# tonyzyl/ladcast

Hardware: AMD Instinct MI355X
Metric: ensemble-member-steps/sec (higher is better)
Workload: dtype f32

## Files before the change

### ladcast_amd/csrc/gemm_bf16x3_v3.hip

```cpp
#include <math.h>
#include <stdio.h>
#include <stdlib.h>

#include "common.h"

namespace {

#include "gemm_v3_common.inc"
#include "gemm_v3_kstep_f32.inc"

struct SKArgs {
  DevProblem pr[MAXP];
  int np;
  int G;
  long long U;
  long long tiles;
  float* ws;
  unsigned* counters;
  unsigned upg, urem;
};

__device__ __forceinline__ long long range_start(long long g, const SKArgs& a) {
  const unsigned gu = static_cast<unsigned>(g);
  return static_cast<long long>(gu * a.upg + (gu < a.urem ? gu : a.urem));
}

__device__ __forceinline__ int find_problem_by_unit(const SKArgs& a, long long u) {
  int pi = 0;
#pragma unroll
  for (int k = 1; k < MAXP; ++k)
    if (k < a.np && u >= a.pr[k].unit0) pi = k;
  return pi;
}

#ifdef LDC_GEMM_STAMPS
#define LDC_STAMP(i)                                                                                        \
  if (threadIdx.x == 0)                                                                                     \
    reinterpret_cast<unsigned long long*>(a.counters)[65536 + blockIdx.x * 16 + (i)] = __builtin_amdgcn_s_memrealtime();
#define LDC_STAMP_CLK(i)                                                                                    \
  if (threadIdx.x == 0)                                                                                     \
    reinterpret_cast<unsigned long long*>(a.counters)[65536 + blockIdx.x * 16 + (i)] = __builtin_amdgcn_s_memtime();
#else
#define LDC_STAMP(i)
#define LDC_STAMP_CLK(i)
#endif

template <int BM, int TERMS, bool CONV = false>
__global__ __launch_bounds__(512) void gemm_bf16x3_v3_kernel(SKArgs a) {
  constexpr int CPK = TERMS == 1 ? 2 * BK : BK;
  constexpr int RT = BM / 128;
  constexpr int NACC = RT * 8;
  constexpr int STAGE_B = (BM + BN) * ROW_B;
  constexpr int SLOT_FLOATS = BM * BN;
  constexpr int NAI = BM / 64;
  constexpr int ND = NAI + 2;
  constexpr int NDH = ND / 2;
  extern __shared__ __attribute__((aligned(16))) unsigned char smem[];
  const int wave = __builtin_amdgcn_readfirstlane(static_cast<int>(threadIdx.x) >> 6);
  LDC_STAMP(0)
  int seg_ = 0;
  (void)seg_;
  int g;
  {
    const int bid = blockIdx.x, G = a.G;
    const int q = G >> 3, r = G & 7, xcd = bid & 7;
    g = (xcd < r ? xcd * (q + 1) : r * (q + 1) + (xcd - r) * q) + (bid >> 3);
  }
  auto uniform64 = [](long long v) {
    const unsigned lo = __builtin_amdgcn_readfirstlane(static_cast<unsigned>(v));
    const unsigned hi = __builtin_amdgcn_readfirstlane(static_cast<unsigned>(static_cast<unsigned long long>(v) >> 32));
    return static_cast<long long>((static_cast<unsigned long long>(hi) << 32) | lo);
  };
  const long long u_begin = uniform64(range_start(g, a));
  const long long u_end = uniform64(range_start(g + 1, a));
  const unsigned smem_lds = lds_addr(smem);

  struct Seg {
    int pi, tile, k0, k1, b, bm, bn;
  };
  auto decode = [&](long long u_) {
    Seg sg;
    sg.pi = find_problem_by_unit(a, u_);
    const DevProblem& Q = a.pr[sg.pi];
    const unsigned local = static_cast<unsigned>(u_ - Q.unit0), kt_u = static_cast<unsigned>(Q.kt);
    sg.tile = __builtin_amdgcn_readfirstlane(static_cast<int>(local / kt_u));
    sg.k0 = static_cast<int>(local - static_cast<unsigned>(sg.tile) * kt_u);
    const long long left = u_end - u_;
    sg.k1 = (Q.kt - sg.k0 <= left) ? Q.kt : sg.k0 + static_cast<int>(left);
    const unsigned per_b = static_cast<unsigned>(Q.tm * Q.tn), tile_u = static_cast<unsigned>(sg.tile);
    const unsigned b_ = tile_u / per_b;
    const unsigned t_in = tile_u - b_ * per_b;
    const unsigned strip = static_cast<unsigned>(Q.rm * Q.tn);
    const unsigned sr = t_in / strip;
    const unsigned r_in = t_in - sr * strip;
    const int rest = Q.tm - static_cast<int>(sr) * Q.rm;
    const unsigned h_sr = static_cast<unsigned>(rest < Q.rm ? rest : Q.rm);
    const unsigned bn_ = r_in / h_sr;
    sg.b = __builtin_amdgcn_readfirstlane(static_cast<int>(b_));
    sg.bn = __builtin_amdgcn_readfirstlane(static_cast<int>(bn_));
    sg.bm = __builtin_amdgcn_readfirstlane(static_cast<int>(sr) * Q.rm + static_cast<int>(r_in - bn_ * h_sr));
    return sg;
  };
  auto prefetch_next = [&](const Seg& sg) __attribute__((always_inline)) {
    const DevProblem& Q = a.pr[sg.pi];
    const int ln = fresh_lane();
    const int lr_ = ln >> 3, lp_ = ln & 7;
    const float* __restrict__ An = Q.A + static_cast<long long>(sg.b) * Q.d.a_bs;
    const long long wrb = static_cast<long long>(Q.d.K) * (TERMS == 1 ? 2 : 4);
    unsigned char* dump = smem + NSTAGE * STAGE_B + wave * 1024;
#pragma unroll
    for (int j = 0; j < 2; ++j) {
      const bool live = sg.k0 + j < sg.k1;
      const long long koff = static_cast<long long>(live ? sg.k0 + j : sg.k1 - 1) * (BK * 4);
      unsigned char* sA = smem + j * STAGE_B;
      unsigned char* sW = sA + BM * ROW_B;
#pragma unroll
      for (int i = 0; i < NAI; ++i) {
        const int r = 8 * (wave + 8 * i) + lr_;
        int gm = sg.bm * BM + r;
        gm = gm < Q.d.M ? gm : Q.d.M - 1;
        dma16(reinterpret_cast<const unsigned char*>(An + static_cast<long long>(gm) * Q.d.lda) + ((lp_ ^ swz(r)) << 4) + koff,
              live ? sA + (wave + 8 * i) * 1024 : dump);
      }
#pragma unroll
      for (int i = 0; i < 2; ++i) {
        const int r = 8 * (wave + 8 * i) + lr_;
        int gn = sg.bn * BN + r;
        gn = gn < Q.d.N ? gn : Q.d.N - 1;
        dma16(Q.W + static_cast<long long>(gn) * wrb + ((lp_ ^ swz(r)) << 4) + koff, live ? sW + (wave + 8 * (i)) * 1024 : dump);
      }
    }
  };
  long long u = u_begin;
  Seg cur{};
  if (u < u_end) cur = decode(u);
  bool prefetched = false;
  while (u < u_end) {
    const int pi = cur.pi;
    const DevProblem& P = a.pr[pi];
    const int tile = cur.tile, k0 = cur.k0, k1 = cur.k1, b = cur.b, bm = cur.bm, bn = cur.bn;
    const int lane = fresh_lane();
    const int fr = lane & 15;
    const int kg = lane >> 4;
    const int lr = lane >> 3, lp = lane & 7;
    const unsigned f_r = swz(fr);
    const unsigned off_hi = fr * ROW_B + (((2 * kg) ^ f_r) << 4);
    const unsigned off_lo = fr * ROW_B + (((2 * kg + 1) ^ f_r) << 4);
    const unsigned a_hi = smem_lds + (16 * RT * wave) * ROW_B + off_hi;
    const unsigned a_lo = smem_lds + (16 * RT * wave) * ROW_B + off_lo;
    const unsigned w_hi = smem_lds + BM * ROW_B + off_hi;
    const unsigned w_lo = smem_lds + BM * ROW_B + off_lo;
    const int M = P.d.M, N = P.d.N, K = P.d.K;
    const bool wave_rows = bm * BM + 16 * RT * wave < M;
    const float* __restrict__ A = P.A + static_cast<long long>(b) * P.d.a_bs;
    const int lda = P.d.lda;
    const long long w_row_bytes = static_cast<long long>(K) * (TERMS == 1 ? 2 : 4);

#ifdef LDC_GEMM_STAMPS_PROLOGUE
    if (seg_ == 0) { LDC_STAMP(9) }
#endif
    const unsigned char* a_src[NAI];
    const unsigned char* w_src[2];
    int pix_b[NAI], pix_hw[NAI];
    const int cslot = lp ^ swz(8 * (wave & 1) + lr);
    auto conv_tap_base = [&](int i, int tap) {
      const int ky = tap / P.ks, kx = tap - ky * P.ks;
      const int src = pix_b[i] + ldc_sphere_src_pixel(pix_hw[i] >> 16, pix_hw[i] & 0xffff, ky, kx, P.cH, P.cW, P.ks);
      return reinterpret_cast<const unsigned char*>(A + static_cast<long long>(src) * lda) + (cslot << 4);
    };
#pragma unroll
    for (int i = 0; i < NAI; ++i) {
      const int r = 8 * (wave + 8 * i) + lr;
      int gm = bm * BM + r;
      gm = gm < M ? gm : M - 1;
      if constexpr (CONV) {
        const int hw = P.cH * P.cW;
        const int bimg = gm / hw;
        const int rem = gm - bimg * hw;
        const int h = rem / P.cW;
        pix_b[i] = bimg * hw;
        pix_hw[i] = (h << 16) | (rem - h * P.cW);
        a_src[i] = conv_tap_base(i, k0 >> P.kshift);
      } else {
        a_src[i] = reinterpret_cast<const unsigned char*>(A + static_cast<long long>(gm) * lda) + ((lp ^ swz(r)) << 4);
      }
    }
#pragma unroll
    for (int i = 0; i < 2; ++i) {
      const int r = 8 * (wave + 8 * i) + lr;
      int gn = bn * BN + r;
      gn = gn < N ? gn : N - 1;
      w_src[i] = P.W + static_cast<long long>(gn) * w_row_bytes + ((lp ^ swz(r)) << 4);
    }
    auto issue_one = [&](int kt_, int stage, int i) {
      const bool live = kt_ < k1;
      unsigned char* sA = smem + stage * STAGE_B;
      unsigned char* sW = sA + BM * ROW_B;
      unsigned char* dump = smem + NSTAGE * STAGE_B + wave * 1024;
      const int kt = live ? kt_ : k1 - 1;
      const long long koff = static_cast<long long>(kt) * (BK * 4);
#ifdef LDC_GEMM_DIAG_NODMA
      if (kt >= 0) return;
#endif
      if (i < NAI) {
        if constexpr (CONV) {
          const int chunk = kt & ((1 << P.kshift) - 1);
          if (chunk == 0) a_src[i] = conv_tap_base(i, kt >> P.kshift);
          const unsigned char* src = a_src[i] + chunk * (BK * 4);
          if (chunk * CPK + CPK > P.cin) {
            if (chunk * CPK + (TERMS == 0 ? 4 * cslot : 8 * (TERMS == 3 ? (cslot >> 1) : cslot)) >= P.cin) src = P.zero16;
          }
          dma16(src, live ? sA + (wave + 8 * i) * 1024 : dump);
        } else {
          dma16(a_src[i] + koff, live ? sA + (wave + 8 * i) * 1024 : dump);
        }
      } else {
        dma16(w_src[i - NAI] + koff, live ? sW + (wave + 8 * (i - NAI)) * 1024 : dump);
      }
    };

    f32x4 acc[NACC];
#pragma unroll
    for (int i = 0; i < NACC; ++i) acc[i] = f32x4{0.f, 0.f, 0.f, 0.f};

    i32x4v wh0, wl0, wh1, wl1, wh2, wl2, wh3, wl3;
    i32x4v ah0[RT], al0[RT], ah1[RT], al1[RT];

#define LDC_SB __builtin_amdgcn_sched_barrier(0)
#define LDC_RD_W(WH, WL, SBH, SBL, CT)                                           \
  {                                                                              \
    LDC_DS_READ(WH, SBH, (CT) * (16 * ROW_B));                                   \
    LDC_DS_READ(WL, SBL, (CT) * (16 * ROW_B));                                   \
  }
#define LDC_RD_A(AH, AL, SBH, SBL)                                               \
  {                                                                              \
    LDC_DS_READ(AH[0], SBH, 0);                                                  \
    LDC_DS_READ(AL[0], SBL, 0);                                                  \
    if constexpr (RT == 2) {                                                     \
      LDC_DS_READ(AH[RT - 1], SBH, 16 * ROW_B);                                  \
      LDC_DS_READ(AL[RT - 1], SBL, 16 * ROW_B);                                  \
    }                                                                            \
  }
#define LDC_MM(ACC, WF, AF)                                                                                  \
  ACC = __builtin_amdgcn_mfma_f32_16x16x32_bf16(__builtin_bit_cast(bf16x8, WF), __builtin_bit_cast(bf16x8, AF), ACC, 0, 0, 0); \
  LDC_SB;
#define LDC_MMF(ACC, WF, AF, J)                                                                               \
  ACC = __builtin_amdgcn_mfma_f32_16x16x4f32(__int_as_float(WF[J]), __int_as_float(AF[J]), ACC, 0, 0, 0);     \
  LDC_SB;
#define LDC_CT(CT, WH, WL, AH, AL)                                               \
  if (wave_rows) {                                                               \
    if constexpr (TERMS == 0) {                                                  \
      _Pragma("unroll") for (int j_ = 0; j_ < 4; ++j_) {                         \
        LDC_MMF(acc[(CT)], WH, AH[0], j_)                                        \
        if constexpr (RT == 2) {                                                 \
          LDC_MMF(acc[8 + (CT)], WH, AH[RT - 1], j_)                             \
        }                                                                        \
      }                                                                          \
      _Pragma("unroll") for (int j_ = 0; j_ < 4; ++j_) {                         \
        LDC_MMF(acc[(CT)], WL, AL[0], j_)                                        \
        if constexpr (RT == 2) {                                                 \
          LDC_MMF(acc[8 + (CT)], WL, AL[RT - 1], j_)                             \
        }                                                                        \
      }                                                                          \
    } else if constexpr (TERMS == 1) {                                           \
      LDC_MM(acc[(CT)], WH, AH[0])                                               \
      if constexpr (RT == 2) {                                                   \
        LDC_MM(acc[8 + (CT)], WH, AH[RT - 1])                                    \
      }                                                                          \
      LDC_MM(acc[(CT)], WL, AL[0])                                               \
      if constexpr (RT == 2) {                                                   \
        LDC_MM(acc[8 + (CT)], WL, AL[RT - 1])                                    \
      }                                                                          \
    } else if constexpr (RT == 2) {                                              \
      LDC_MM(acc[(CT)], WH, AL[0])                                               \
      LDC_MM(acc[8 + (CT)], WH, AL[RT - 1])                                      \
      LDC_MM(acc[(CT)], WL, AH[0])                                               \
      LDC_MM(acc[8 + (CT)], WL, AH[RT - 1])                                      \
      LDC_MM(acc[(CT)], WH, AH[0])                                               \
      LDC_MM(acc[8 + (CT)], WH, AH[RT - 1])                                      \
    } else {                                                                     \
      LDC_MM(acc[(CT)], WH, AL[0])                                               \
      LDC_MM(acc[(CT)], WL, AH[0])                                               \
      LDC_MM(acc[(CT)], WH, AH[0])                                               \
    }                                                                            \
  }
#ifdef LDC_GEMM_DIAG_NOBARRIER
#define LDC_KSTEP_BARRIER
#else
#define LDC_KSTEP_BARRIER __builtin_amdgcn_s_barrier();
#endif
#define LDC_WAIT(N, X, Y)                                                        \
  asm volatile("s_waitcnt lgkmcnt(6)" : "+v"(X), "+v"(Y));                       \
  LDC_SB;
#define LDC_KSTEP(AH, AL, AHN, ALN)                                                                          \
  {                                                                                                          \
    const int st1 = st == NSTAGE - 1 ? 0 : st + 1;                                                           \
    const int st2 = st1 == NSTAGE - 1 ? 0 : st1 + 1;                                                         \
    const unsigned sb1 = st1 * STAGE_B;                                                                      \
    const unsigned wch = w_hi + sb, wcl = w_lo + sb, wnh = w_hi + sb1, wnl = w_lo + sb1;                     \
    const unsigned anh = a_hi + sb1, anl = a_lo + sb1;                                                       \
    constexpr bool dma2 = true;              \
    constexpr bool dma3 = true;  \
        \
    if constexpr (RT == 2) {                                                                                 \
      asm volatile("s_waitcnt lgkmcnt(6)" : "+v"(AH[0]), "+v"(AL[0]), "+v"(AH[1]), "+v"(AL[1]), "+v"(wh0), "+v"(wl0)); \
    } else {                                                                                                 \
      asm volatile("s_waitcnt lgkmcnt(6)" : "+v"(AH[0]), "+v"(AL[0]), "+v"(wh0), "+v"(wl0));                 \
    }                                                                                                        \
    LDC_SB;                                                                                                  \
    LDC_CT(0, wh0, wl0, AH, AL)                                                                              \
    LDC_RD_W(wh0, wl0, wch, wcl, 4)                                                                                \
    if (dma2) issue_one(kt + 2, st2, NDH + 0);                                                               \
    LDC_WAIT(6, wh1, wl1)                                                                                    \
    LDC_CT(1, wh1, wl1, AH, AL)                                                                              \
    LDC_RD_W(wh1, wl1, wch, wcl, 5)                                                                                \
    if (dma2) issue_one(kt + 2, st2, NDH + 1);                                                               \
    LDC_WAIT(6, wh2, wl2)                                                                                    \
    LDC_CT(2, wh2, wl2, AH, AL)                                                                              \
    LDC_RD_W(wh2, wl2, wch, wcl, 6)                                                                                \
    if constexpr (NDH == 3) {                                                                                \
      if (dma2) issue_one(kt + 2, st2, NDH + 2);                                                             \
    }                                                                                                        \
    LDC_WAIT(6, wh3, wl3)                                                                                    \
    LDC_CT(3, wh3, wl3, AH, AL)                                                                              \
    LDC_RD_W(wh3, wl3, wch, wcl, 7)                                                                          \
    LDC_WAIT(6, wh0, wl0)                                                                                    \
    LDC_CT(4, wh0, wl0, AH, AL)                                                                              \
                                                                         \
    asm volatile("s_waitcnt lgkmcnt(0)" : "+v"(wh1), "+v"(wl1), "+v"(wh2), "+v"(wl2), "+v"(wh3), "+v"(wl3)); \
    if constexpr (ND == 6) {                                                                                 \
      asm volatile("s_waitcnt vmcnt(6)" ::: "memory");                                                       \
    } else {                                                                                                 \
      asm volatile("s_waitcnt vmcnt(4)" ::: "memory");                                                       \
    }                                                                                                        \
    LDC_KSTEP_BARRIER                                                                                        \
    LDC_SB;                                                                                                  \
                          \
    LDC_RD_A(AHN, ALN, anh, anl)                                                                             \
    LDC_RD_W(wh0, wl0, wnh, wnl, 0)                                                                          \
    if (dma3) issue_one(kt + 3, st, 0);                                                                      \
    LDC_SB;                                                                                                  \
    LDC_CT(5, wh1, wl1, AH, AL)                                                                              \
    LDC_RD_W(wh1, wl1, wnh, wnl, 1)                                                                               \
    if (dma3) issue_one(kt + 3, st, 1);                                                                      \
    LDC_SB;                                                                                                  \
    LDC_CT(6, wh2, wl2, AH, AL)                                                                              \
    LDC_RD_W(wh2, wl2, wnh, wnl, 2)                                                                               \
    if constexpr (NDH == 3) {                                                                                \
      if (dma3) issue_one(kt + 3, st, 2);                                                                    \
    }                                                                                                        \
    LDC_SB;                                                                                                  \
    LDC_CT(7, wh3, wl3, AH, AL)                                                                              \
    LDC_RD_W(wh3, wl3, wnh, wnl, 3)                                                                               \
    LDC_SB;                                                                                                  \
    st = st1;                                                                                                \
    sb = sb1;                                                                                                \
  }

#define LDC_MM_ON(ACC, WF, AF, J) LDC_MMF(ACC, WF, AF, J)
#define LDC_MM_OFF(ACC, WF, AF, J)
#if defined(LDC_AB_BUILD) && defined(LDC_GEMM_F32_NO_PAIRS)
  constexpr bool PAIRED = false;
#else
  constexpr bool PAIRED = TERMS == 0 && RT == 1;
#endif

#ifdef LDC_GEMM_STAMPS_PROLOGUE
    if (seg_ == 0) { LDC_STAMP(10) }
#endif
    if (!prefetched) {
#pragma unroll
      for (int i = 0; i < ND; ++i) issue_one(k0, 0, i);
#pragma unroll
      for (int i = 0; i < ND; ++i) issue_one(k0 + 1, 1, i);
    }
#ifdef LDC_GEMM_STAMPS_PROLOGUE
    if (seg_ == 0) { LDC_STAMP(11) }
#endif
    const long long u_next = u + (k1 - k0);
    Seg nxt = cur;
    if (u_next < u_end) nxt = decode(u_next);
    if constexpr (ND == 6) {
      asm volatile("s_waitcnt vmcnt(6)" ::: "memory");
    } else {
      asm volatile("s_waitcnt vmcnt(4)" ::: "memory");
    }
    __builtin_amdgcn_s_barrier();
    LDC_STAMP(1 + 4 * seg_)
    if (seg_ == 0) { LDC_STAMP_CLK(13) }
    if constexpr (PAIRED) {
      LDC_KSTEP_Q_PROLOGUE(ah0, al0)
    } else {
      LDC_RD_A(ah0, al0, a_hi, a_lo)
      LDC_RD_W(wh0, wl0, w_hi, w_lo, 0)
      LDC_RD_W(wh1, wl1, w_hi, w_lo, 1)
      LDC_RD_W(wh2, wl2, w_hi, w_lo, 2)
      LDC_RD_W(wh3, wl3, w_hi, w_lo, 3)
    }
#pragma unroll
    for (int i = 0; i < NDH; ++i) issue_one(k0 + 2, 2, i);
    LDC_SB;

    unsigned sb = 0;
    int st = 0;
    if constexpr (PAIRED) {
      static_assert(!PAIRED || ND == 4, "the interleaved k-step is written for the 128-row tile's 4 DMA pieces");
      if (wave_rows) {
        for (int kt = k0; kt < k1; ++kt) {
          LDC_KSTEP_Q(ah0, al0, ah1, al1, LDC_MM_ON)
          ++kt;
          if (kt >= k1) break;
          LDC_KSTEP_Q(ah1, al1, ah0, al0, LDC_MM_ON)
        }
      } else {
        for (int kt = k0; kt < k1; ++kt) {
          LDC_KSTEP_Q(ah0, al0, ah1, al1, LDC_MM_OFF)
          ++kt;
          if (kt >= k1) break;
          LDC_KSTEP_Q(ah1, al1, ah0, al0, LDC_MM_OFF)
        }
      }
    } else {
      for (int kt = k0; kt < k1; ++kt) {
        LDC_KSTEP(ah0, al0, ah1, al1)
        ++kt;
        if (kt >= k1) break;
        LDC_KSTEP(ah1, al1, ah0, al0)
      }
    }
    asm volatile("s_waitcnt lgkmcnt(0)" : "+v"(wh0), "+v"(wl0), "+v"(wh1), "+v"(wl1), "+v"(wh2), "+v"(wl2), "+v"(wh3), "+v"(wl3));
#pragma unroll
    for (int rt = 0; rt < RT; ++rt) asm volatile("" : "+v"(ah0[rt]), "+v"(al0[rt]), "+v"(ah1[rt]), "+v"(al1[rt]));
#undef LDC_KSTEP
#undef LDC_MM_ON
#undef LDC_MM_OFF
#undef LDC_WAIT
#undef LDC_CT
#undef LDC_MMF
#undef LDC_MM
#undef LDC_RD_A
#undef LDC_RD_W
#undef LDC_SB
    __builtin_amdgcn_s_barrier();
    prefetched = false;
    if constexpr (!CONV && TERMS == 0) {
#if !defined(LDC_GEMM_DIAG_NODMA) && !defined(LDC_GEMM_NO_PREFETCH)
      if (u_next < u_end) {
        prefetch_next(nxt);
        prefetched = true;
      }
#endif
    }
    if (seg_ == 0) { LDC_STAMP_CLK(14) }
    LDC_STAMP(2 + 4 * seg_)

    if (k0 == 0 && k1 == P.kt) {
      tile_epilogue<BM, !CONV, LinearRows<BM>, true, TERMS == 0>(P, b, bm, bn, acc, wave, lane);
    } else {
      const int lane_h = fresh_lane();
      float* slot = a.ws + (static_cast<long long>(2 * g) + (k0 > 0 ? 0 : 1)) * SLOT_FLOATS + lane_h;
#pragma unroll
      for (int i = 0; i < NACC; ++i)
#pragma unroll
        for (int r = 0; r < 4; ++r)
          __hip_atomic_store(slot + ((wave * NACC + i) * 4 + r) * 64, acc[i][r], __ATOMIC_RELAXED, __HIP_MEMORY_SCOPE_AGENT);
      asm volatile("s_waitcnt vmcnt(0)" ::: "memory");
      __builtin_amdgcn_s_barrier();
      const long long f = P.unit0 + static_cast<long long>(tile) * P.kt;
      const long long l = f + P.kt;
      long long g_first = g;
      while (g_first > 0 && range_start(g_first, a) > f) --g_first;
      long long g_last = g;
      while (g_last + 1 < a.G && range_start(g_last + 1, a) < l) ++g_last;
      const unsigned pieces = static_cast<unsigned>(g_last - g_first + 1);
      unsigned* cnt = a.counters + (P.tile0 + tile);
      unsigned* flag = reinterpret_cast<unsigned*>(smem + NSTAGE * STAGE_B);
      if (wave == 0 && lane_h == 0) {
        const unsigned ticket = __hip_atomic_fetch_add(cnt, 1u, __ATOMIC_RELAXED, __HIP_MEMORY_SCOPE_AGENT);
        const unsigned last = (ticket == pieces - 1) ? 1u : 0u;
        if (last) {
          __builtin_amdgcn_fence(__ATOMIC_ACQUIRE, "agent");
          asm volatile("s_waitcnt vmcnt(0)" ::: "memory");
          __hip_atomic_store(cnt, 0u, __ATOMIC_RELAXED, __HIP_MEMORY_SCOPE_AGENT);
        }
        *flag = last;
      }
      __syncthreads();
      LDC_STAMP(3 + 4 * seg_)
      const unsigned is_last = *flag;
      __syncthreads();
      if (is_last) {
#pragma unroll
        for (int i = 0; i < NACC; ++i) acc[i] = f32x4{0.f, 0.f, 0.f, 0.f};
        for (long long gp = g_first; gp <= g_last; ++gp) {
          const long long s = range_start(gp, a);
          const float* sl = a.ws + (2 * gp + (s > f ? 0 : 1)) * SLOT_FLOATS;
#pragma unroll
          for (int i = 0; i < NACC; ++i) {
#pragma unroll
            for (int r = 0; r < 4; ++r) acc[i][r] += sl[((wave * NACC + i) * 4 + r) * 64 + lane_h];
          }
        }
        tile_epilogue<BM, !CONV, LinearRows<BM>, true, TERMS == 0>(P, b, bm, bn, acc, wave, lane);
      }
    }
    u = u_next;
    cur = nxt;
    LDC_STAMP(4 + 4 * seg_)
#ifdef LDC_GEMM_STAMPS
    if (seg_ < 2) ++seg_;
#endif
  }
  LDC_STAMP(15)
}

template <int BM, int TERMS, bool CONV = false>
int launch_v3(const ldc_gemm_problem* problems, int n, const ldc_gemm_launch_plan& plan, const ldc_conv_params* cp, void* workspace,
              void* stream) {
  constexpr int STAGE_B = (BM + BN) * ROW_B;
  SKArgs a{};
  a.np = n;
  for (int i = 0; i < n; ++i) {
    const ldc_gemm_problem& q = problems[i];
    const ldc_gemm_problem_plan& pp = plan.pr[i];
    DevProblem& P = a.pr[i];
    P.A = q.A;
    P.W = reinterpret_cast<const unsigned char*>(q.W);
    P.bias = q.bias;
    P.gate = q.gate;
    P.R = q.R;
    P.C = q.C;
    P.d = q.d;
    P.tm = pp.tm; P.tn = pp.tn; P.kt = pp.kt; P.rm = pp.rm;
    P.unit0 = pp.unit0;
    P.tile0 = pp.tile0;
    P.vec4 = pp.vec4;
    P.c_split = pp.c_split;
    P.qkv_heads = pp.qkv_heads;
    P.rope_row0 = pp.rope_row0;
    P.qk_w[0] = pp.qk_w[0];
    P.qk_w[1] = pp.qk_w[1];
    P.rope_cs = pp.rope_cs;
    P.eps = pp.eps;
    P.qscale = pp.qscale;
    if constexpr (CONV) {
      P.cH = cp->H; P.cW = cp->W; P.cin = cp->cin; P.ks = cp->ks; P.kshift = cp->kshift;
      P.zero16 = static_cast<const unsigned char*>(workspace) + LDC_GEMM_COUNTER_BYTES - 64;
    }
  }
  a.G = plan.G;
  a.U = plan.U;
  a.upg = plan.upg;
  a.urem = plan.urem;
  a.tiles = plan.tiles;
  a.ws = reinterpret_cast<float*>(static_cast<unsigned char*>(workspace) + LDC_GEMM_COUNTER_BYTES);
  a.counters = static_cast<unsigned*>(workspace);
  const size_t lds = NSTAGE * STAGE_B + 8 * 1024;
  static const bool attr_set = [&] {
    (void)hipFuncSetAttribute(reinterpret_cast<const void*>(gemm_bf16x3_v3_kernel<BM, TERMS, CONV>),
                              hipFuncAttributeMaxDynamicSharedMemorySize, static_cast<int>(lds));
    return true;
  }();
  (void)attr_set;
  hipLaunchKernelGGL((gemm_bf16x3_v3_kernel<BM, TERMS, CONV>), dim3(a.G), dim3(512), lds, static_cast<hipStream_t>(stream), a);
  return ldc_launch_status();
}

}

int ldc_gemm_ring_launch(const ldc_gemm_problem* problems, int n, const ldc_gemm_launch_plan& plan, int bm, int terms,
                         const ldc_conv_params* cp, void* workspace, void* stream) {
  const bool sm = bm == 128;
  if (cp == nullptr) {
    if (terms == 1)
      return sm ? launch_v3<128, 1>(problems, n, plan, cp, workspace, stream) : launch_v3<256, 1>(problems, n, plan, cp, workspace, stream);
    if (terms == 3)
      return sm ? launch_v3<128, 3>(problems, n, plan, cp, workspace, stream) : launch_v3<256, 3>(problems, n, plan, cp, workspace, stream);
#ifdef LDC_AB_BUILD
    if (!sm) return launch_v3<256, 0>(problems, n, plan, cp, workspace, stream);
#endif
    return launch_v3<128, 0>(problems, n, plan, cp, workspace, stream);
  }
  if (terms == 0) return launch_v3<128, 0, true>(problems, n, plan, cp, workspace, stream);
  if (terms == 1)
    return sm ? launch_v3<128, 1, true>(problems, n, plan, cp, workspace, stream) : launch_v3<256, 1, true>(problems, n, plan, cp, workspace, stream);
  return sm ? launch_v3<128, 3, true>(problems, n, plan, cp, workspace, stream) : launch_v3<256, 3, true>(problems, n, plan, cp, workspace, stream);
}

extern "C" int ldc_sphere_conv_nhwc_split(const float* X, const void* Wp, const float* bias, const float* R, float* Y, int B, int H,
                                          int W, int cin, int ldx, int cout, int ldy, int ldr, int ksize, int act, int in_fmt,
                                          int out_fmt, void* workspace, long long workspace_bytes, void* stream) {
  LDC_CHECK_PTR(X);
  LDC_CHECK_PTR(Wp);
  LDC_CHECK_PTR(Y);
  if (B <= 0 || H <= 0 || W <= 0 || cin <= 0 || cout <= 0) return LDC_ERR_ARG;
  if (ksize != 1 && ksize != 3 && ksize != 5) return LDC_ERR_UNSUPPORTED;
  if (ksize > 1 && ((W & 1) || H < 2 || H < ksize / 2 || W / 2 < ksize / 2 || H > 32767 || W > 65535)) return LDC_ERR_UNSUPPORTED;
  if (in_fmt != LDC_FMT_SPLIT && in_fmt != LDC_FMT_BF16 && in_fmt != LDC_FMT_F32) return LDC_ERR_UNSUPPORTED;
  if (out_fmt != LDC_FMT_F32 && out_fmt != in_fmt) return LDC_ERR_UNSUPPORTED;
  if (in_fmt == LDC_FMT_F32) {
    if ((ldx & 3) || (cin & 3) || ldx < cin || ldy < cout) return LDC_ERR_ALIGN;
  } else if ((ldx & 7) || ldx < ((cin + 7) & ~7) || ldy < cout) {
    return LDC_ERR_ALIGN;
  }
  const long long M = static_cast<long long>(B) * H * W;
  if (M > 0x7fffffffLL) return LDC_ERR_UNSUPPORTED;
  const bool one = in_fmt == LDC_FMT_BF16;
  const int cpk = one ? 2 * BK : BK;
  ldc_conv_params cp{H, W, cin, ksize, 0};
  int ktpt = ldc_cdiv(cin, cpk);
  while ((1 << cp.kshift) < ktpt) ++cp.kshift;
  ktpt = 1 << cp.kshift;
  ldc_gemm_problem q{};
  q.A = X;
  q.W = static_cast<const float*>(Wp);
  q.bias = bias;
  q.R = R;
  q.C = Y;
  q.d.M = static_cast<int>(M);
  q.d.N = cout;
  q.d.K = ksize * ksize * ktpt * cpk;
  q.d.batch = 1;
  q.d.lda = ldx;
  q.d.ldw = q.d.K;
  q.d.ldc = ldy;
  q.d.ldr = ldr;
  q.d.act = act;
  q.d.flags = LDC_GEMM_A_SPLIT | (out_fmt != LDC_FMT_F32 ? LDC_GEMM_C_SPLIT : 0) | (one ? LDC_GEMM_BF16_1TERM : 0);
  auto run = [&](int bm, int terms) {
    ldc_gemm_launch_plan plan;
    const int st = ldc_gemm_plan_ring(&q, nullptr, 1, workspace, workspace_bytes, bm, terms, &cp, &plan);
    return st != LDC_OK ? st : ldc_gemm_ring_launch(&q, 1, plan, bm, terms, &cp, workspace, stream);
  };
  if (in_fmt == LDC_FMT_F32) {
    q.d.flags = 0;
    return run(128, 0);
  }
  if (ksize == 3) {
    static const char* const halo_sw = LDC_AB_GETENV("LDC_CONV_HALO");
    if (!(halo_sw && atoi(halo_sw) == 0)) {
      if (workspace == nullptr || workspace_bytes < LDC_GEMM_COUNTER_BYTES) return LDC_ERR_ARG;
      const int hs = ldc_conv_halo_dispatch(X, Wp, bias, R, Y, B, H, W, cin, ldx, cout, ldy, ldr, act, in_fmt, out_fmt, workspace, workspace_bytes, stream);
      if (hs != LDC_ERR_UNSUPPORTED) return hs;
    }
  }
  const long long tiles256 = static_cast<long long>(ldc_cdiv(M, 256)) * ldc_cdiv(cout, BN);
  static const char* const force_thr = LDC_AB_GETENV("LDC_CONV_SMALL_TILES");
  const bool small = tiles256 < (force_thr ? atoll(force_thr) : 200);
  return run(small ? 128 : 256, one ? 1 : 3);
}
```

Before: 3.240.

## Add no-copy interleaved f32 k-step that rotates weight registers without copies

Adds a new paired f32 k-step for the non-conv TERMS==0, RT==1 path. It rotates LDS reads through the weight fragment registers in place, so register-to-register copies between k-steps go away and the next step's reads and DMA issues interleave more tightly with the MFMA sequence. It also adds a drain step at loop exit and a build flag that restricts launches to the f32 instances. The risk is extra register pressure, plus scheduling fragility from the hand-placed waitcnt counts.

```diff
diff --git a/ladcast_amd/csrc/gemm_bf16x3_v3.hip b/ladcast_amd/csrc/gemm_bf16x3_v3.hip
--- a/ladcast_amd/csrc/gemm_bf16x3_v3.hip
+++ b/ladcast_amd/csrc/gemm_bf16x3_v3.hip
@@ -8,6 +8,7 @@
 
 #include "gemm_v3_common.inc"
 #include "gemm_v3_kstep_f32.inc"
+#include "gemm_v3_kstep_f32_nocopy.inc"
 
 struct SKArgs {
   DevProblem pr[MAXP];
@@ -364,6 +365,7 @@
 #else
   constexpr bool PAIRED = TERMS == 0 && RT == 1;
 #endif
+  constexpr bool NOCOPY = PAIRED && !CONV;
 
 #ifdef LDC_GEMM_STAMPS_PROLOGUE
     if (seg_ == 0) { LDC_STAMP(10) }
@@ -388,7 +390,8 @@
     __builtin_amdgcn_s_barrier();
     LDC_STAMP(1 + 4 * seg_)
     if (seg_ == 0) { LDC_STAMP_CLK(13) }
-    if constexpr (PAIRED) {
+    if constexpr (NOCOPY) {
+    } else if constexpr (PAIRED) {
       LDC_KSTEP_Q_PROLOGUE(ah0, al0)
     } else {
       LDC_RD_A(ah0, al0, a_hi, a_lo)
@@ -403,7 +406,30 @@
 
     unsigned sb = 0;
     int st = 0;
-    if constexpr (PAIRED) {
+    if constexpr (NOCOPY) {
+      static_assert(!NOCOPY || ND == 4, "the interleaved k-step is written for the 128-row tile's 4 DMA pieces");
+#define LDC_KSTEP_QC_DRAIN(AH, AL)                                                                                                      \
+  asm volatile("s_waitcnt lgkmcnt(0)" ::"v"(AH[0]), "v"(AL[0]), "v"(wh0), "v"(wl0), "v"(wh1), "v"(wl1), "v"(wh2), "v"(wh3));          \
+  LDC_SB;
+      if (wave_rows) {
+        LDC_KSTEP_QC_PROLOGUE(ah0, al0)
+        for (int kt = k0;;) {
+          LDC_KSTEP_QC(ah0, al0, ah1, al1, LDC_MM_ON)
+          if (++kt >= k1) { LDC_KSTEP_QC_DRAIN(ah1, al1) break; }
+          LDC_KSTEP_QC(ah1, al1, ah0, al0, LDC_MM_ON)
+          if (++kt >= k1) { LDC_KSTEP_QC_DRAIN(ah0, al0) break; }
+        }
+      } else {
+        LDC_KSTEP_QC_PROLOGUE(ah0, al0)
+        for (int kt = k0;;) {
+          LDC_KSTEP_QC(ah0, al0, ah1, al1, LDC_MM_OFF)
+          if (++kt >= k1) { LDC_KSTEP_QC_DRAIN(ah1, al1) break; }
+          LDC_KSTEP_QC(ah1, al1, ah0, al0, LDC_MM_OFF)
+          if (++kt >= k1) { LDC_KSTEP_QC_DRAIN(ah0, al0) break; }
+        }
+      }
+#undef LDC_KSTEP_QC_DRAIN
+    } else if constexpr (PAIRED) {
       static_assert(!PAIRED || ND == 4, "the interleaved k-step is written for the 128-row tile's 4 DMA pieces");
       if (wave_rows) {
         for (int kt = k0; kt < k1; ++kt) {
@@ -428,9 +454,11 @@
         LDC_KSTEP(ah1, al1, ah0, al0)
       }
     }
-    asm volatile("s_waitcnt lgkmcnt(0)" : "+v"(wh0), "+v"(wl0), "+v"(wh1), "+v"(wl1), "+v"(wh2), "+v"(wl2), "+v"(wh3), "+v"(wl3));
-#pragma unroll
-    for (int rt = 0; rt < RT; ++rt) asm volatile("" : "+v"(ah0[rt]), "+v"(al0[rt]), "+v"(ah1[rt]), "+v"(al1[rt]));
+    if constexpr (!NOCOPY) {
+      asm volatile("s_waitcnt lgkmcnt(0)" : "+v"(wh0), "+v"(wl0), "+v"(wh1), "+v"(wl1), "+v"(wh2), "+v"(wl2), "+v"(wh3), "+v"(wl3));
+#pragma unroll
+      for (int rt = 0; rt < RT; ++rt) asm volatile("" : "+v"(ah0[rt]), "+v"(al0[rt]), "+v"(ah1[rt]), "+v"(al1[rt]));
+    }
 #undef LDC_KSTEP
 #undef LDC_MM_ON
 #undef LDC_MM_OFF
@@ -571,6 +599,10 @@
 int ldc_gemm_ring_launch(const ldc_gemm_problem* problems, int n, const ldc_gemm_launch_plan& plan, int bm, int terms,
                          const ldc_conv_params* cp, void* workspace, void* stream) {
   const bool sm = bm == 128;
+#ifdef LDC_GEMM_F32_INSTANCES_ONLY
+  if (terms != 0 || !sm) return LDC_ERR_UNSUPPORTED;
+  return cp == nullptr ? launch_v3<128, 0>(problems, n, plan, cp, workspace, stream) : launch_v3<128, 0, true>(problems, n, plan, cp, workspace, stream);
+#else
   if (cp == nullptr) {
     if (terms == 1)
       return sm ? launch_v3<128, 1>(problems, n, plan, cp, workspace, stream) : launch_v3<256, 1>(problems, n, plan, cp, workspace, stream);
@@ -585,6 +617,7 @@
   if (terms == 1)
     return sm ? launch_v3<128, 1, true>(problems, n, plan, cp, workspace, stream) : launch_v3<256, 1, true>(problems, n, plan, cp, workspace, stream);
   return sm ? launch_v3<128, 3, true>(problems, n, plan, cp, workspace, stream) : launch_v3<256, 3, true>(problems, n, plan, cp, workspace, stream);
+#endif
 }
 
 extern "C" int ldc_sphere_conv_nhwc_split(const float* X, const void* Wp, const float* bias, const float* R, float* Y, int B, int H,
diff --git a/ladcast_amd/csrc/gemm_v3_kstep_f32_nocopy.inc b/ladcast_amd/csrc/gemm_v3_kstep_f32_nocopy.inc
--- /dev/null
+++ b/ladcast_amd/csrc/gemm_v3_kstep_f32_nocopy.inc
@@ -0,0 +1,141 @@
+#define LDC_KSTEP_QC(AH, AL, AHN, ALN, MM) \
+  { \
+    const int st1 = st == NSTAGE - 1 ? 0 : st + 1; \
+    const int st2 = st1 == NSTAGE - 1 ? 0 : st1 + 1; \
+    (void)st2; \
+    const unsigned sb1 = st1 * STAGE_B; \
+    const unsigned wch = w_hi + sb, wcl = w_lo + sb, wnh = w_hi + sb1, wnl = w_lo + sb1; \
+    const unsigned anh = a_hi + sb1, anl = a_lo + sb1; \
+    asm volatile("s_waitcnt lgkmcnt(2)" :: "v"(AH[0]), "v"(AL[0]), "v"(wh0), "v"(wl0), "v"(wh1), "v"(wl1)); \
+    LDC_SB; \
+    MM(acc[0], wh0, AH[0], 0) \
+    LDC_DS_READ(wl2, wcl, 2 * (16 * ROW_B)); \
+    LDC_SB; \
+    MM(acc[1], wh1, AH[0], 0) \
+    MM(acc[0], wh0, AH[0], 1) \
+    LDC_DS_READ(wl3, wcl, 3 * (16 * ROW_B)); \
+    LDC_SB; \
+    MM(acc[1], wh1, AH[0], 1) \
+    MM(acc[0], wh0, AH[0], 2) \
+    MM(acc[1], wh1, AH[0], 2) \
+    MM(acc[0], wh0, AH[0], 3) \
+    MM(acc[1], wh1, AH[0], 3) \
+    MM(acc[0], wl0, AL[0], 0) \
+    LDC_DS_READ(wh0, wch, 4 * (16 * ROW_B)); \
+    LDC_SB; \
+    MM(acc[1], wl1, AL[0], 0) \
+    MM(acc[0], wl0, AL[0], 1) \
+    LDC_DS_READ(wh1, wch, 5 * (16 * ROW_B)); \
+    LDC_SB; \
+    MM(acc[1], wl1, AL[0], 1) \
+    MM(acc[0], wl0, AL[0], 2) \
+    issue_one(kt + 2, st2, NDH + 0); \
+    LDC_SB; \
+    MM(acc[1], wl1, AL[0], 2) \
+    MM(acc[0], wl0, AL[0], 3) \
+    issue_one(kt + 2, st2, NDH + 1); \
+    LDC_SB; \
+    MM(acc[1], wl1, AL[0], 3) \
+    asm volatile("s_waitcnt lgkmcnt(2)" :: "v"(wh2), "v"(wh3), "v"(wl2), "v"(wl3)); \
+    LDC_SB; \
+    MM(acc[2], wh2, AH[0], 0) \
+    LDC_DS_READ(wl0, wcl, 4 * (16 * ROW_B)); \
+    LDC_SB; \
+    MM(acc[3], wh3, AH[0], 0) \
+    MM(acc[2], wh2, AH[0], 1) \
+    LDC_DS_READ(wl1, wcl, 5 * (16 * ROW_B)); \
+    LDC_SB; \
+    MM(acc[3], wh3, AH[0], 1) \
+    MM(acc[2], wh2, AH[0], 2) \
+    MM(acc[3], wh3, AH[0], 2) \
+    MM(acc[2], wh2, AH[0], 3) \
+    MM(acc[3], wh3, AH[0], 3) \
+    MM(acc[2], wl2, AL[0], 0) \
+    LDC_DS_READ(wh2, wch, 6 * (16 * ROW_B)); \
+    LDC_SB; \
+    MM(acc[3], wl3, AL[0], 0) \
+    MM(acc[2], wl2, AL[0], 1) \
+    LDC_DS_READ(wh3, wch, 7 * (16 * ROW_B)); \
+    LDC_SB; \
+    MM(acc[3], wl3, AL[0], 1) \
+    MM(acc[2], wl2, AL[0], 2) \
+    MM(acc[3], wl3, AL[0], 2) \
+    MM(acc[2], wl2, AL[0], 3) \
+    MM(acc[3], wl3, AL[0], 3) \
+    asm volatile("s_waitcnt lgkmcnt(2)" :: "v"(wh0), "v"(wh1), "v"(wl0), "v"(wl1)); \
+    LDC_SB; \
+    MM(acc[4], wh0, AH[0], 0) \
+    LDC_DS_READ(wl2, wcl, 6 * (16 * ROW_B)); \
+    LDC_SB; \
+    MM(acc[5], wh1, AH[0], 0) \
+    MM(acc[4], wh0, AH[0], 1) \
+    LDC_DS_READ(wl3, wcl, 7 * (16 * ROW_B)); \
+    LDC_SB; \
+    MM(acc[5], wh1, AH[0], 1) \
+    MM(acc[4], wh0, AH[0], 2) \
+    MM(acc[5], wh1, AH[0], 2) \
+    MM(acc[4], wh0, AH[0], 3) \
+    MM(acc[5], wh1, AH[0], 3) \
+    MM(acc[4], wl0, AL[0], 0) \
+    MM(acc[5], wl1, AL[0], 0) \
+    MM(acc[4], wl0, AL[0], 1) \
+    MM(acc[5], wl1, AL[0], 1) \
+    MM(acc[4], wl0, AL[0], 2) \
+    MM(acc[5], wl1, AL[0], 2) \
+    MM(acc[4], wl0, AL[0], 3) \
+    MM(acc[5], wl1, AL[0], 3) \
+     \
+    asm volatile("s_waitcnt lgkmcnt(0)" :: "v"(wh2), "v"(wh3), "v"(wl2), "v"(wl3)); \
+    asm volatile("s_waitcnt vmcnt(4)" ::: "memory"); \
+    LDC_KSTEP_BARRIER \
+    LDC_SB; \
+    MM(acc[6], wh2, AH[0], 0) \
+    LDC_DS_READ(AHN[0], anh, 0 * (16 * ROW_B)); \
+    LDC_SB; \
+    MM(acc[7], wh3, AH[0], 0) \
+    LDC_DS_READ(ALN[0], anl, 0 * (16 * ROW_B)); \
+    LDC_SB; \
+    MM(acc[6], wh2, AH[0], 1) \
+    LDC_DS_READ(wh0, wnh, 0 * (16 * ROW_B)); \
+    LDC_SB; \
+    MM(acc[7], wh3, AH[0], 1) \
+    LDC_DS_READ(wl0, wnl, 0 * (16 * ROW_B)); \
+    LDC_SB; \
+    MM(acc[6], wh2, AH[0], 2) \
+    LDC_DS_READ(wh1, wnh, 1 * (16 * ROW_B)); \
+    LDC_SB; \
+    MM(acc[7], wh3, AH[0], 2) \
+    LDC_DS_READ(wl1, wnl, 1 * (16 * ROW_B)); \
+    LDC_SB; \
+    MM(acc[6], wh2, AH[0], 3) \
+    issue_one(kt + 3, st, 0); \
+    LDC_SB; \
+    MM(acc[7], wh3, AH[0], 3) \
+    issue_one(kt + 3, st, 1); \
+    LDC_SB; \
+    MM(acc[6], wl2, AL[0], 0) \
+    LDC_DS_READ(wh2, wnh, 2 * (16 * ROW_B)); \
+    LDC_SB; \
+    MM(acc[7], wl3, AL[0], 0) \
+    MM(acc[6], wl2, AL[0], 1) \
+    LDC_DS_READ(wh3, wnh, 3 * (16 * ROW_B)); \
+    LDC_SB; \
+    MM(acc[7], wl3, AL[0], 1) \
+    MM(acc[6], wl2, AL[0], 2) \
+    MM(acc[7], wl3, AL[0], 2) \
+    MM(acc[6], wl2, AL[0], 3) \
+    MM(acc[7], wl3, AL[0], 3) \
+    st = st1; \
+    sb = sb1; \
+  }
+#define LDC_KSTEP_QC_PROLOGUE(AH, AL) \
+  { \
+    LDC_DS_READ(AH[0], a_hi, 0 * (16 * ROW_B)); \
+    LDC_DS_READ(AL[0], a_lo, 0 * (16 * ROW_B)); \
+    LDC_DS_READ(wh0, w_hi, 0 * (16 * ROW_B)); \
+    LDC_DS_READ(wl0, w_lo, 0 * (16 * ROW_B)); \
+    LDC_DS_READ(wh1, w_hi, 1 * (16 * ROW_B)); \
+    LDC_DS_READ(wl1, w_lo, 1 * (16 * ROW_B)); \
+    LDC_DS_READ(wh2, w_hi, 2 * (16 * ROW_B)); \
+    LDC_DS_READ(wh3, w_hi, 3 * (16 * ROW_B)); \
+  }
```

Result: faster. 3.281 (median of 6 runs) (+1.3%).
